# freewym/espresso

Hardware: AMD Instinct MI355X
Metric: audio-hours/sec training (LibriSpeech Conformer-12 + CTC) (higher is better)
Workload: dtype bf16

## Files before the change

espresso_amd/csrc/conv_igemm.hip:

```cpp
#include <hip/hip_runtime.h>

#include "gemm_common.h"

namespace {

typedef const __attribute__((address_space(1))) void* gptr_t;
typedef __attribute__((address_space(3))) void* lptr_t;

struct ConvGatherArgs {
  const bf16_t* src;
  const bf16_t* W;
  bf16_t* out;
  const float* bias;
  double* stats;
  const bf16_t* zero;
  int RB, RT, RF;
  int ST, SF, SC;
  int at, af;
  int ntaps;
  int bt[9], bf[9], koff[9];
  int N;
  long ldw;
  int OT, OF, ot_mul, ot_add, of_mul, of_add;
};

template <int BN_>
__global__ __launch_bounds__(256, 2) void conv_gather_kernel(const ConvGatherArgs a) {
  constexpr int BM_ = 128, NST = 2;
  constexpr int NJ = BN_ / 32;
  constexpr int A_BYTES = BM_ * ROW_BYTES, STAGE = A_BYTES + BN_ * ROW_BYTES;
  constexpr int NA = BM_ / 32, NB = BN_ / 32;
  extern __shared__ __attribute__((aligned(16))) char dsm[];
  const int tid = threadIdx.x, lane = tid & 63, wave = tid >> 6;
  const int wm = wave >> 1, wcol = (wave & 1) * (BN_ / 2);
  const uint32_t M = (uint32_t)a.RB * a.RT * a.RF;
  const uint32_t m0 = blockIdx.x * BM_;
  const int cpt = a.SC / BK;
  const int nk = a.ntaps * cpt;

  int rowb[NA], rowt[NA], rowf[NA];
  int cs[NA];
#pragma unroll
  for (int i = 0; i < NA; ++i) {
    const int r = (wave + 4 * i) * 8 + (lane >> 3);
    cs[i] = (lane & 7) ^ (r & 7) ^ ((r >> 4) & 7);
    const uint32_t p = m0 + r;
    if (p < M) {
      const uint32_t q = p / (uint32_t)a.RF, b = q / (uint32_t)a.RT;
      const int rf = (int)(p - q * a.RF), rt = (int)(q - b * a.RT);
      rowb[i] = (int)b * a.ST;
      rowt[i] = rt * a.at;
      rowf[i] = rf * a.af;
    } else {
      rowb[i] = -1;
      rowt[i] = rowf[i] = 0;
    }
  }
  const bf16_t* bp[NB];
#pragma unroll
  for (int i = 0; i < NB; ++i) {
    const int r = (wave + 4 * i) * 8 + (lane >> 3);
    const int c = (lane & 7) ^ (r & 7) ^ ((r >> 4) & 7);
    bp[i] = a.W + (long)min(r, a.N - 1) * a.ldw + c * 8;
  }
  auto issue = [&](int stage, int kt) {
    const int tap = kt / cpt, chunk = kt - tap * cpt;
    const int dt = a.bt[tap], df = a.bf[tap];
    const long ko = a.koff[tap] + chunk * BK;
    char* base = dsm + stage * STAGE + wave * 1024;
#pragma unroll
    for (int i = 0; i < NA; ++i) {
      const int st = rowt[i] + dt, sf = rowf[i] + df;
      const bool ok = rowb[i] >= 0 && (unsigned)st < (unsigned)a.ST && (unsigned)sf < (unsigned)a.SF;
      const bf16_t* s = ok ? a.src + (((long)(rowb[i] + st)) * a.SF + sf) * a.SC + chunk * BK + cs[i] * 8 : a.zero + cs[i] * 8;
      __builtin_amdgcn_global_load_lds((gptr_t)s, (lptr_t)(base + i * 4096), 16, 0, 0);
    }
#pragma unroll
    for (int i = 0; i < NB; ++i)
      __builtin_amdgcn_global_load_lds((gptr_t)(bp[i] + ko), (lptr_t)(base + A_BYTES + i * 4096), 16, 0, 0);
  };

  f32x4_t acc[4][NJ];
#pragma unroll
// ... 27 lines not shown
      for (int i = 0; i < 4; ++i)
#pragma unroll
        for (int j = 0; j < NJ; ++j)
          acc[i][j] = __builtin_amdgcn_mfma_f32_16x16x32_bf16(
              __builtin_bit_cast(__attribute__((ext_vector_type(8))) __bf16, af[i]),
              __builtin_bit_cast(__attribute__((ext_vector_type(8))) __bf16, bfr[j]), acc[i][j], 0, 0, 0);
    }
    stage ^= 1;
  }

  constexpr int CG = BN_ / 8;
  constexpr int RL = 256 / CG;
  float* sC = reinterpret_cast<float*>(dsm);
  const int cg = tid % CG, rlane = tid / CG;
  float bias8[8], s8[8], q8[8];
#pragma unroll
  for (int e = 0; e < 8; ++e) {
    bias8[e] = a.bias ? a.bias[cg * 8 + e] : 0.f;
    s8[e] = q8[e] = 0.f;
  }
#pragma unroll 1
  for (int half = 0; half < 2; ++half) {
    __syncthreads();
    if (wm == half) {
#pragma unroll
      for (int i = 0; i < 4; ++i)
#pragma unroll
        for (int j = 0; j < NJ; ++j)
#pragma unroll
          for (int r = 0; r < 4; ++r) sC[(i * 16 + (lane >> 4) * 4 + r) * BN_ + wcol + j * 16 + (lane & 15)] = acc[i][j][r];
    }
    __syncthreads();
#pragma unroll 1
    for (int pass = 0; pass < 64 / RL; ++pass) {
      const int rl = pass * RL + rlane;
      const uint32_t p = m0 + half * 64 + rl;
      if (p < M) {
        const uint32_t q = p / (uint32_t)a.RF, b = q / (uint32_t)a.RT;
        const int rf = (int)(p - q * a.RF), rt = (int)(q - b * a.RT);
        const long orow = ((long)b * a.OT + (long)rt * a.ot_mul + a.ot_add) * a.OF + (long)rf * a.of_mul + a.of_add;
        const float4 x0 = *reinterpret_cast<const float4*>(sC + rl * BN_ + cg * 8);
        const float4 x1 = *reinterpret_cast<const float4*>(sC + rl * BN_ + cg * 8 + 4);
        float v[8] = {x0.x, x0.y, x0.z, x0.w, x1.x, x1.y, x1.z, x1.w};
#pragma unroll
        for (int e = 0; e < 8; ++e) v[e] += bias8[e];
        uint4 u;
        u.x = pack_bf2(v[0], v[1]); u.y = pack_bf2(v[2], v[3]); u.z = pack_bf2(v[4], v[5]); u.w = pack_bf2(v[6], v[7]);
        *reinterpret_cast<uint4*>(a.out + orow * a.N + cg * 8) = u;
        if (a.stats) {
          const uint32_t w[4] = {u.x, u.y, u.z, u.w};
#pragma unroll
          for (int e = 0; e < 4; ++e) {
            const float lo = __uint_as_float(w[e] << 16), hi = __uint_as_float(w[e] & 0xffff0000u);
            s8[2 * e] += lo; q8[2 * e] += lo * lo;
            s8[2 * e + 1] += hi; q8[2 * e + 1] += hi * hi;
          }
        }
      }
    }
  }
  if (a.stats) {
    __syncthreads();
    float* red = reinterpret_cast<float*>(dsm);
#pragma unroll
    for (int e = 0; e < 8; ++e) {
      red[(rlane * 2 + 0) * BN_ + cg * 8 + e] = s8[e];
      red[(rlane * 2 + 1) * BN_ + cg * 8 + e] = q8[e];
    }
    __syncthreads();
    if (tid < 2 * BN_) {
      const int which = tid / BN_, c = tid - which * BN_;
      float t = 0.f;
      for (int r = 0; r < RL; ++r) t += red[(r * 2 + which) * BN_ + c];
      atomicAdd(a.stats + which * a.N + c, (double)t);
    }
  }
}

const bf16_t* zero_line(hipStream_t stream) {
  static bf16_t* z = nullptr;
  if (!z) {
    if (hipMalloc(&z, 256) != hipSuccess) return nullptr;
    if (hipMemsetAsync(z, 0, 256, stream) != hipSuccess) return nullptr;
    hipStreamSynchronize(stream);
  }
  return z;
}

template <int BN_>
int launch_gather(const ConvGatherArgs& a, hipStream_t stream) {
  constexpr int bytes = 2 * (128 + BN_) * ROW_BYTES;
  static bool attr_ok = hipFuncSetAttribute(reinterpret_cast<const void*>(&conv_gather_kernel<BN_>),
                                            hipFuncAttributeMaxDynamicSharedMemorySize, bytes) == hipSuccess;
  if (!attr_ok) return -1;
  const long M = (long)a.RB * a.RT * a.RF;
  if (M <= 0) return 0;
  if (M >= (1L << 31) - 128) return -1;
  hipLaunchKernelGGL((conv_gather_kernel<BN_>), dim3((unsigned)((M + 127) / 128)), dim3(256), bytes, stream, a);
  return EA_CHECK_LAUNCH();
}


struct ConvWgradArgs {
  const bf16_t* X;
  const bf16_t* dZ;
  float* slab;
  const bf16_t* zero;
  int RB, RT, RF, ST, SF, Cin, Cout;
  int at, af, ntaps;
  int bt[9], bf[9];
  int chunks_per_wg;
  int ablate;
};

__device__ __forceinline__ int tr_sw(int r) { return (r & 3) ^ ((r >> 3) & 1); }
__device__ __forceinline__ void ds_read_tr16_x8(const uint32_t (&ad)[8], uint2 (&o)[8]) {
// ... 209 lines not shown
  const long chunks = (M + 63) / 64;
  const int blocks = (Cin / 64) * (Cout / 64);
  static const long target = [] { const char* e = getenv("EA_CONV_WGRAD_WGS"); const long v = e ? atol(e) : 0; return v > 0 ? v : 256L; }();
  long nsplit = (target + blocks - 1) / blocks;
  if (nsplit > chunks / 8) nsplit = chunks / 8;
  if (nsplit < 1) nsplit = 1;
  return (int)nsplit;
}

}

extern "C" int ea_conv3x3_fwd(const void* X, const void* W, const float* bias, void* Z, double* stats, int B, int T, int F,
                              int Cin, int Cout, int sy, int sx, hipStream_t stream) {
  if (B <= 0 || T <= 0 || F <= 0) return 0;
  if (Cin % 64 || (Cout != 64 && Cout != 128) || sy < 1 || sx < 1) return -2;
  ConvGatherArgs a;
  a.src = (const bf16_t*)X; a.W = (const bf16_t*)W; a.out = (bf16_t*)Z; a.bias = bias; a.stats = stats;
  a.zero = zero_line(stream);
  if (!a.zero) return -1;
  const int To = (T - 1) / sy + 1, Fo = (F - 1) / sx + 1;
  a.RB = B; a.RT = To; a.RF = Fo;
  a.ST = T; a.SF = F; a.SC = Cin;
  a.at = sy; a.af = sx;
  a.ntaps = 9;
  for (int ky = 0; ky < 3; ++ky)
    for (int kx = 0; kx < 3; ++kx) {
      const int t = ky * 3 + kx;
      a.bt[t] = ky - 1; a.bf[t] = kx - 1; a.koff[t] = t * Cin;
    }
  a.N = Cout; a.ldw = 9L * Cin;
  a.OT = To; a.OF = Fo; a.ot_mul = 1; a.ot_add = 0; a.of_mul = 1; a.of_add = 0;
  return Cout == 128 ? launch_gather<128>(a, stream) : launch_gather<64>(a, stream);
}

extern "C" int ea_conv3x3_dgrad(const void* dZ, const void* Wd, void* dX, int B, int T, int F, int Cin, int Cout, int sy, int sx,
                                hipStream_t stream) {
  if (B <= 0 || T <= 0 || F <= 0) return 0;
  if (Cout % 64 || (Cin != 64 && Cin != 128) || sy < 1 || sx < 1 || sy > 2 || sx > 2) return -2;
  const int To = (T - 1) / sy + 1, Fo = (F - 1) / sx + 1;
  const bf16_t* zero = zero_line(stream);
  if (!zero) return -1;
  for (int pt = 0; pt < sy; ++pt)
    for (int pf = 0; pf < sx; ++pf) {
      ConvGatherArgs a;
      a.src = (const bf16_t*)dZ; a.W = (const bf16_t*)Wd; a.out = (bf16_t*)dX; a.bias = nullptr; a.stats = nullptr; a.zero = zero;
      a.RB = B; a.RT = (T - pt + sy - 1) / sy; a.RF = (F - pf + sx - 1) / sx;
      a.ST = To; a.SF = Fo; a.SC = Cout;
      a.at = 1; a.af = 1;
      a.ntaps = 0;
      for (int ky = 0; ky < 3; ++ky) {
        if ((pt + 1 - ky) % sy) continue;
        for (int kx = 0; kx < 3; ++kx) {
          if ((pf + 1 - kx) % sx) continue;
          const int t = a.ntaps++;
          a.bt[t] = (pt + 1 - ky) / sy; a.bf[t] = (pf + 1 - kx) / sx; a.koff[t] = (ky * 3 + kx) * Cout;
        }
      }
      a.N = Cin; a.ldw = 9L * Cout;
      a.OT = T; a.OF = F; a.ot_mul = sy; a.ot_add = pt; a.of_mul = sx; a.of_add = pf;
      if (a.RT <= 0 || a.RF <= 0) continue;
      if (a.ntaps == 0) return -2;
      const int rc = Cin == 128 ? launch_gather<128>(a, stream) : launch_gather<64>(a, stream);
      if (rc) return rc;
    }
  return 0;
}

extern "C" long ea_conv3x3_wgrad_workspace_bytes(int B, int T, int F, int Cin, int Cout, int sy, int sx) {
  const int To = (T - 1) / sy + 1, Fo = (F - 1) / sx + 1;
  return (long)wgrad_split((long)B * To * Fo, Cin, Cout) * Cout * 9 * Cin * (long)sizeof(float);
}

static int conv3x3_wgrad_impl(const void* X, const void* dZ, float* dW, void* workspace, int B, int T, int F, int Cin, int Cout,
                              int sy, int sx, int param_layout, hipStream_t stream);
extern "C" int ea_conv3x3_wgrad(const void* X, const void* dZ, float* dW, void* workspace, int B, int T, int F, int Cin, int Cout,
                                int sy, int sx, hipStream_t stream) {
  return conv3x3_wgrad_impl(X, dZ, dW, workspace, B, T, F, Cin, Cout, sy, sx, 0, stream);
}
extern "C" int ea_conv3x3_wgrad_param_layout(const void* X, const void* dZ, float* dW, void* workspace, int B, int T, int F, int Cin,
                                             int Cout, int sy, int sx, hipStream_t stream) {
  return conv3x3_wgrad_impl(X, dZ, dW, workspace, B, T, F, Cin, Cout, sy, sx, 1, stream);
// ... 40 lines not shown
```

espresso_amd/csrc/convmodule.hip:

```cpp
#include "common.h"
#include "espresso_amd.h"

namespace {

constexpr int KMAX = 31;

__device__ __forceinline__ float sigmoid_f(float x) { return __builtin_amdgcn_rcpf(1.f + __expf(-x)); }

constexpr int CT = 64, TTILE = 64, TPT = TTILE / 4;

template <int KW>
__global__ __launch_bounds__(256) void glu_dwconv_fwd_kernel(const bf16_t* __restrict__ Y,
                                                             const float* __restrict__ w,
                                                             bf16_t* __restrict__ U, bf16_t* __restrict__ Z,
                                                             double* __restrict__ stats, int T, int C) {
  constexpr int PAD = (KW - 1) / 2, ROWS = TTILE + KW - 1;
  __shared__ __attribute__((aligned(16))) float su[ROWS][CT];
  __shared__ float sred[2][4][CT];
  const int c0 = blockIdx.x * CT, t0 = blockIdx.y * TTILE, b = blockIdx.z;
  const long rowbase = (long)b * T;
  if ((C & 7) == 0 && c0 + CT <= C) {
    bf16_t (*sub)[CT] = reinterpret_cast<bf16_t (*)[CT]>(&su[0][0]);
    bf16_t (*sz)[CT] = reinterpret_cast<bf16_t (*)[CT]>(&su[0][0]) + ROWS;
    constexpr int NCH = (ROWS * (CT / 8) + 255) / 256;
// ... 733 lines not shown
__device__ __forceinline__ int c1_sw(int r) { return (r & 3) ^ ((r >> 3) & 1); }
__device__ __forceinline__ void c1_tr_read8(const uint32_t (&ad)[8], uint2 (&o)[8]) {
  asm volatile(
      "ds_read_b64_tr_b16 %0, %8\n\tds_read_b64_tr_b16 %1, %9\n\tds_read_b64_tr_b16 %2, %10\n\tds_read_b64_tr_b16 %3, %11\n\t"
      "ds_read_b64_tr_b16 %4, %12\n\tds_read_b64_tr_b16 %5, %13\n\tds_read_b64_tr_b16 %6, %14\n\tds_read_b64_tr_b16 %7, %15\n\t"
      "s_waitcnt lgkmcnt(0)"
      : "=&v"(o[0]), "=&v"(o[1]), "=&v"(o[2]), "=&v"(o[3]), "=&v"(o[4]), "=&v"(o[5]), "=&v"(o[6]), "=&v"(o[7])
      : "v"(ad[0]), "v"(ad[1]), "v"(ad[2]), "v"(ad[3]), "v"(ad[4]), "v"(ad[5]), "v"(ad[6]), "v"(ad[7])
      : "memory");
}
__global__ __launch_bounds__(256) void conv1_bn_bwd_wgrad_kernel(const float* __restrict__ X, const bf16_t* __restrict__ Z,
                                                                 const bf16_t* __restrict__ dH, const float* __restrict__ mean_rstd,
                                                                 const float* __restrict__ gamma, const float* __restrict__ beta,
                                                                 const float* __restrict__ red, float* __restrict__ dW,
                                                                 float* __restrict__ dbias, int T, int F, int To, int Fo, int CO,
                                                                 int sy, int sx, long npos, int act, float n) {
  __shared__ __attribute__((aligned(16))) char tile[4][32 * 128];
  __shared__ float sred[4][64][16];
  const int lane = threadIdx.x & 63, wave = threadIdx.x >> 6;
  const int li = lane & 15, g4 = lane >> 4;
  const float invn = n > 0.f ? 1.f / n : 0.f;
  const long nblk = (npos + 31) / 32;
  const long bmax = (npos - 1) / ((long)Fo * To);
  const uint32_t lds0 = (uint32_t)(uintptr_t)(&tile[wave][0]);
  for (int cs = 0; cs < CO; cs += 64) {
    const int c8 = lane & 7, prow = lane >> 3;
    float mu[8], rs[8], ga[8], be[8], r0[8], r1[8];
#pragma unroll
    for (int e = 0; e < 8; ++e) {
      const int c = cs + c8 * 8 + e;
      mu[e] = mean_rstd[c]; rs[e] = mean_rstd[CO + c]; ga[e] = gamma[c]; be[e] = beta[c];
      r0[e] = red[c] * invn; r1[e] = red[CO + c] * invn;
    }
    f32x4_t acc[4];
// ... 141 lines not shown
                               int F, int CO, int sy, int sx, int act, int training, hipStream_t stream) {
  if (B <= 0 || T <= 0) return 0;
  if (CO % 64) return -2;
  const int To = (T - 1) / sy + 1, Fo = (F - 1) / sx + 1;
  const long npos = (long)B * To * Fo;
  launch_bn_bwd_reduce(Z, dH, mean_rstd, gamma, beta, red, npos, CO, act, stream);
  long nb = (npos + 127) / 128;
  if (nb > 1024) nb = 1024;
  hipLaunchKernelGGL(conv1_bn_bwd_wgrad_kernel, dim3((unsigned)nb), dim3(256), 0, stream, X, (const bf16_t*)Z,
                     (const bf16_t*)dH, mean_rstd, gamma, beta, red, dW, dbias, T, F, To, Fo, CO, sy, sx, npos, act,
                     training ? (float)npos : 0.f);
  if (dgamma || dbeta) hipLaunchKernelGGL(bn_param_grad_kernel, dim3((CO + 255) / 256), dim3(256), 0, stream, red, dgamma, dbeta, CO);
  return EA_CHECK_LAUNCH();
}

static void launch_bn_bwd_reduce(const void* Z, const void* dH, const float* mean_rstd, const float* gamma, const float* beta,
                                 float* red, long M, int C, int act, hipStream_t stream) {
  const int nch = C / 8;
  int TCH = 1;
  while (TCH < 256 && TCH < nch) TCH <<= 1;
  const int lanes = 256 / TCH;
  int rpb = 8 * lanes;
  if (rpb < 32) rpb = 32;
  const long gx = (nch + TCH - 1) / TCH;
  const long want = (M + (2048 / gx) - 1) / (2048 / gx > 0 ? 2048 / gx : 1);
  if (want > rpb) rpb = (int)((want + lanes - 1) / lanes * lanes);
  dim3 g1((unsigned)gx, (unsigned)((M + rpb - 1) / rpb));
  hipLaunchKernelGGL(bn_act_bwd_reduce_kernel, g1, dim3(256), (size_t)256 * 16 * sizeof(float), stream, (const bf16_t*)Z,
                     (const bf16_t*)dH, mean_rstd, gamma, beta, red, M, C, act, rpb, TCH);
}
// ... 53 lines not shown
```

espresso_amd/functional.py:

```python
import collections

import ctypes
import os

import torch

from . import kernels as K

_seed_state = {"base": 0x5EED, "counter": 0}


def set_dropout_seed(seed: int):
    _seed_state["base"] = int(seed) & 0xFFFFFFFF
    _seed_state["counter"] = 0


_seed_trace = None


class trace_dropout_seeds:

    def __enter__(self):
        global _seed_trace
        self.prev, self.entries = _seed_trace, []
# ... 641 lines not shown
    return _LabelSmoothedCE.apply(logits, target, pad_idx, eps, smoothing, prior, tgt_len)


_CONV_IGEMM = True


_CONV1_FUSED_BWD = True


def set_conv1_fused_backward(on: bool) -> bool:
    global _CONV1_FUSED_BWD
    old, _CONV1_FUSED_BWD = _CONV1_FUSED_BWD, bool(on)
    return old


def set_conv_implicit_gemm(on: bool):
    global _CONV_IGEMM
    _CONV_IGEMM = bool(on)


def _conv_igemm_ok(cin, cout, sy, sx):
    return _CONV_IGEMM and cin in (64, 128) and cout in (64, 128) and sy in (1, 2) and sx in (1, 2)


class _ConvSubsample(torch.autograd.Function):

    @staticmethod
    def forward(ctx, X, row_zero, strides, bufs, p_drop, training, bn_eps, bn_momentum, *params):
        B, T, F = X.shape
        L = len(params) // 4
# ... 53 lines not shown
        for i in range(L):
            per.append([next(it) if has else None for has in ctx.layout[i]])
        dout = dout.contiguous()
        if seed:
            dout = K.scale_dropout(dout, a=1.0, drop_p=p_drop, drop_seed=seed)
        elif row_zero is not None:
            dout = dout.clone()
        if row_zero is not None:
            K.zero_rows(dout, row_zero)
        grads = [None] * (4 * L)
        Tc, Fc, Cc, To, Fo, Co, sy, sx = cfgs[-1]
        dA = dout.view(B * To * Fo, Co)
        cur = torch.cuda.current_stream(X.device)
        side = _side_stream(X.device)
        keep = []
        for i in range(L - 1, -1, -1):
            Zi, mr, col, w16, g, beta = per[i]
            Tc, Fc, Cc, To, Fo, Co, sy, sx = cfgs[i]
            pw, pb, pg, pbe = ctx.params[4 * i: 4 * i + 4]
            sg, sbe = (_grad_sink(pg, Co), _grad_sink(pbe, Co)) if training else (None, None)
            if sg is not None and sbe is not None:
                dg, dbeta = sg, sbe
            else:
                sg = sbe = None
                dg, dbeta = _zeros_f32(Co, X), _zeros_f32(Co, X)
            if i == 0 and Co % 64 == 0 and _CONV1_FUSED_BWD:
                sW, sb = _grad_sink(pw, Co * 9), _grad_sink(pb, Co)
                if sW is not None and sb is not None:
                    db, dW = sb, sW
                else:
                    sW = None
                    db, dW = _zeros_f32(Co, X), _zeros_f32(Co * 9, X)
                K.conv1_bn_bwd(X, Zi, dA, mr, g, beta, dg, dbeta, dW, db, B, Tc, Fc, Co, sy, sx, "relu", training)
                if sW is None:
                    grads[0], grads[1] = dW.view(wshapes[0]), db
                if sg is None:
                    grads[2], grads[3] = dg, dbeta
                continue
            dZ = K.bn_act_bwd(Zi, dA, mr, g, beta, dg, dbeta, "relu", training)
            keep.append(dZ)
            n = B * To * Fo
            db = _zeros_f32(Co, X)
            if i == 0:
                dW = _zeros_f32(Co * 9, X)
                side.wait_stream(cur)
                with torch.cuda.stream(side):
                    K.conv1_wgrad(X, dZ, dW, db, B, Tc, Fc, Co, sy, sx)
                grads[0] = dW.view(wshapes[0])
            elif ctx.igemm[i]:
                sW = _grad_sink(pw, Co * 9 * Cc)
                side.wait_stream(cur)
                if sW is not None:
                    with torch.cuda.stream(side):
                        K.conv3x3_wgrad(col, dZ, sW, B, Tc, Fc, Cc, Co, sy, sx, param_layout=True)
                else:
                    dWp = _zeros_f32(Co * 9 * Cc, X).view(Co, 9 * Cc)
                    with torch.cuda.stream(side):
                        K.conv3x3_wgrad(col, dZ, dWp, B, Tc, Fc, Cc, Co, sy, sx)
                    grads[4 * i] = dWp.view(Co, 3, 3, Cc).permute(0, 3, 1, 2)
                if not training:
                    db = g.detach() * mr[1] * dbeta
                elif _grad_sink(pb, Co) is not None:
                    db = None
                wd16 = K.cast_f32_to_bf16(ctx.weights[i].detach().permute(1, 2, 3, 0).reshape(Cc, 9 * Co).contiguous())
                dA = K.conv3x3_dgrad(dZ, wd16, B, Tc, Fc, Cc, Co, sy, sx)
            else:
                dWp = torch.empty((Co, 9 * Cc), dtype=torch.float32, device=X.device)
                side.wait_stream(cur)
                with torch.cuda.stream(side):
                    _wgrad(dZ, col, n, Co, 9 * Cc, out=dWp)
                    K.colsum(dZ, db, n, Co, Co)
                grads[4 * i] = dWp.view(Co, 3, 3, Cc).permute(0, 3, 1, 2)
                dcol = _new((n, 9 * Cc), torch.bfloat16, X)
                K.gemm(dZ, w16, dcol, n, 9 * Cc, Co, lda=Co, ldb=9 * Cc, ldc=9 * Cc, b_kstrided=True)
                dA = K.col2im3x3(dcol, B, Tc, Fc, Cc, sy, sx)
            grads[4 * i + 1] = db
            if sg is None:
                grads[4 * i + 2] = dg
                grads[4 * i + 3] = dbeta
        cur.wait_stream(side)
# ... 1303 lines not shown
```

espresso_amd/kernels.py:

```python
import ctypes
from typing import Optional

import torch

from . import _lib
from ._lib import EaGemmParams, check

ACT_NONE, ACT_RELU, ACT_SILU = 0, 1, 2
_ACT = {None: 0, "none": 0, "relu": 1, "silu": 2, "swish": 2}


def _stream():
    return ctypes.c_void_p(torch._C._cuda_getCurrentRawStream(torch._C._cuda_getDevice()))


def _p(t: Optional[torch.Tensor]):
    if t is None:
        return None
    if not t.is_cuda:
        raise RuntimeError("espresso_amd kernels need device tensors (no CPU path)")
    return ctypes.c_void_p(t.data_ptr())


def drop_params(p: float):
# ... 325 lines not shown


def conv3x3_fwd(X, W16, bias, B, T, F, Cin, Cout, sy, sx, stats=None):
    To, Fo = (T - 1) // sy + 1, (F - 1) // sx + 1
    Z = torch.empty((B * To * Fo, Cout), dtype=torch.bfloat16, device=X.device)
    check(_lib.lib().ea_conv3x3_fwd(_p(X), _p(W16), _p(bias), _p(Z), _p(stats), B, T, F, Cin, Cout, sy, sx, _stream()), "ea_conv3x3_fwd")
    return Z


def conv3x3_dgrad(dZ, Wd16, B, T, F, Cin, Cout, sy, sx):
    dX = torch.empty((B * T * F, Cin), dtype=torch.bfloat16, device=dZ.device)
    check(_lib.lib().ea_conv3x3_dgrad(_p(dZ), _p(Wd16), _p(dX), B, T, F, Cin, Cout, sy, sx, _stream()), "ea_conv3x3_dgrad")
    return dX


def conv3x3_wgrad(X, dZ, dW, B, T, F, Cin, Cout, sy, sx, param_layout=False):
    lib = _lib.lib()
    nb = lib.ea_conv3x3_wgrad_workspace_bytes(B, T, F, Cin, Cout, sy, sx)
    ws = torch.empty(nb, dtype=torch.uint8, device=X.device)
    fn = lib.ea_conv3x3_wgrad_param_layout if param_layout else lib.ea_conv3x3_wgrad
    check(fn(_p(X), _p(dZ), _p(dW), _p(ws), B, T, F, Cin, Cout, sy, sx, _stream()), "ea_conv3x3_wgrad")
    return dW


def im2col3x3(A, B, T, F, C, sy, sx):
    To, Fo = (T - 1) // sy + 1, (F - 1) // sx + 1
    col = torch.empty(B * To * Fo, 9 * C, dtype=torch.bfloat16, device=A.device)
    check(_lib.lib().ea_im2col3x3(_p(A), _p(col), B, T, F, C, sy, sx, _stream()), "ea_im2col3x3")
    return col

# ... 382 lines not shown
```

include/espresso_amd.h:

```cpp
#ifndef ESPRESSO_AMD_H
#define ESPRESSO_AMD_H

#include <stdint.h>

#ifdef __cplusplus
extern "C" {
#endif

typedef struct ihipStream_t* ea_stream_t;

int ea_version(void);

enum { EA_ACT_NONE = 0, EA_ACT_RELU = 1, EA_ACT_SILU = 2 };

typedef struct EaGemmParams {
  const void* A;
  const void* B;
  void* C;
  void* C2;
  const float* bias;
  const void* resid;
  const void* aux;
  int M, N, K, batch, zdiv;
  int a_kstrided, b_kstrided, c_f32, accumulate, resid_f32, act;
// ... 137 lines not shown
                      void* wgrad_ws, int B, int T, int C, int KW, ea_stream_t stream);
int ea_dwconv_bwd_weight(const void* dZ, const void* U, float* dw, void* wgrad_ws, int B, int T, int C, int KW, ea_stream_t stream);
int ea_bn_act_fwd_train(const void* Z, const double* stats, float* mean_rstd, float* running_mean, float* running_var,
                        const float* gamma, const float* beta, void* H, long M, int C, int act, float n, float eps,
                        float momentum, double* zero_next, int zero_n, ea_stream_t stream);
int ea_bn_act_bwd_fused(const void* Z, const void* dH, const float* mean_rstd, const float* gamma, const float* beta,
                        float* red, void* dZ, float* dgamma, float* dbeta, long M, int C, int act, int training,
                        float* zero_next, int zero_n, ea_stream_t stream);
int ea_bn_glu_dwconv_bwd_fused(const void* Z, const void* dH, const float* mean_rstd, const float* gamma, const float* beta, float* red,
                               void* dZ, float* dgamma, float* dbeta, int act, int training, float* zero_next, int zero_n,
                               const void* Y, const float* w, void* dY, int B, int T, int C, int KW, ea_stream_t stream);
int ea_bn_param_grad(const float* red, float* dgamma, float* dbeta, int C, ea_stream_t stream);
int ea_conv1_bn_bwd(const float* X, const void* Z, const void* dH, const float* mean_rstd, const float* gamma, const float* beta,
                    float* red, float* dgamma, float* dbeta, float* dW, float* dbias, int B, int T, int F, int CO, int sy, int sx,
                    int act, int training, ea_stream_t stream);

int ea_conv1_fwd(const float* X, const float* W, const float* bias, void* Z, double* stats, int B, int T, int F,
                 int CO, int sy, int sx, ea_stream_t stream);
int ea_conv1_wgrad(const float* X, const void* dZ, float* dW, float* dbias, int B, int T, int F, int CO, int sy,
                   int sx, ea_stream_t stream);
int ea_conv3x3_fwd(const void* X, const void* W, const float* bias, void* Z, double* stats, int B, int T, int F, int Cin,
                   int Cout, int sy, int sx, ea_stream_t stream);
int ea_conv3x3_dgrad(const void* dZ, const void* Wd, void* dX, int B, int T, int F, int Cin, int Cout, int sy, int sx,
                     ea_stream_t stream);
long ea_conv3x3_wgrad_workspace_bytes(int B, int T, int F, int Cin, int Cout, int sy, int sx);
int ea_conv3x3_wgrad(const void* X, const void* dZ, float* dW, void* workspace, int B, int T, int F, int Cin, int Cout, int sy,
                     int sx, ea_stream_t stream);
int ea_conv3x3_wgrad_param_layout(const void* X, const void* dZ, float* dW, void* workspace, int B, int T, int F, int Cin, int Cout,
                                  int sy, int sx, ea_stream_t stream);
int ea_im2col3x3(const void* A, void* col, int B, int T, int F, int C, int sy, int sx, ea_stream_t stream);
int ea_col2im3x3(const void* dcol, void* dA, int B, int T, int F, int C, int sy, int sx, ea_stream_t stream);
int ea_colstats_bf16(const void* X, double* stats, long M, int C, ea_stream_t stream);

int ea_log_softmax_f32(const float* in, long ld_in, float* out, long M, int V, ea_stream_t stream);
int ea_log_softmax_bf16(const void* in, long ld_in, float* out, long M, int V, ea_stream_t stream);
long ea_ctc_workspace_bytes(int B, int T, int Lmax);
int ea_ctc_loss(const float* lprobs, const int* targets, const int* in_len, const int* tgt_len, float* nll,
                void* workspace, int B, int T, int V, int Lmax, int blank, ea_stream_t stream);
int ea_ctc_grad(const float* lprobs, const void* workspace, const float* nll, const int* targets,
// ... 195 lines not shown
```

Before: 5.366.

## Fuse BN backward reductions into strided conv dgrad epilogue and single-launch classes

The strided 3x3 dgrad now runs all parity classes in one launch, with the tap-heavy classes placed first, where it used to launch once per class. Its epilogue also computes the next BatchNorm/ReLU backward partial sums (sum of d and d*xhat) from the freshly produced dX and the saved pre-BN activation. A small fold kernel reduces these per-workgroup partials, and the downstream BN backward and conv1 backward kernels reuse the precomputed sums instead of doing a separate reduction pass over memory. This trades extra Z loads and ALU work in the conv epilogue, plus a workspace buffer, for fewer launches and one fewer full read of the activations.

After: 5.378, median of 6. Within noise of the previous version (+0.2%).

```diff
diff --git a/espresso_amd/csrc/conv_igemm.hip b/espresso_amd/csrc/conv_igemm.hip
--- a/espresso_amd/csrc/conv_igemm.hip
+++ b/espresso_amd/csrc/conv_igemm.hip
@@ -6,6 +6,14 @@
 
 typedef const __attribute__((address_space(1))) void* gptr_t;
 typedef __attribute__((address_space(3))) void* lptr_t;
+
+struct ConvClass {
+  int RT, RF;
+  int ntaps;
+  int ot_add, of_add;
+  int blk0;
+  int bt[9], bf[9], koff[9];
+};
 
 struct ConvGatherArgs {
   const bf16_t* src;
@@ -14,14 +22,20 @@
   const float* bias;
   double* stats;
   const bf16_t* zero;
-  int RB, RT, RF;
+  const bf16_t* bn_Z;
+  const float* bn_mr;
+  const float* bn_g;
+  const float* bn_b;
+  float* bn_part;
+  int bn_act;
+  int RB;
   int ST, SF, SC;
   int at, af;
-  int ntaps;
-  int bt[9], bf[9], koff[9];
   int N;
   long ldw;
-  int OT, OF, ot_mul, ot_add, of_mul, of_add;
+  int OT, OF, ot_mul, of_mul;
+  int ncls;
+  ConvClass cls[4];
 };
 
 template <int BN_>
@@ -33,10 +47,15 @@
   extern __shared__ __attribute__((aligned(16))) char dsm[];
   const int tid = threadIdx.x, lane = tid & 63, wave = tid >> 6;
   const int wm = wave >> 1, wcol = (wave & 1) * (BN_ / 2);
-  const uint32_t M = (uint32_t)a.RB * a.RT * a.RF;
-  const uint32_t m0 = blockIdx.x * BM_;
+  int ci = 0;
+  for (int c = 1; c < a.ncls; ++c)
+    if ((int)blockIdx.x >= a.cls[c].blk0) ci = c;
+  const ConvClass& k = a.cls[ci];
+  const int RT = k.RT, RF = k.RF;
+  const uint32_t M = (uint32_t)a.RB * RT * RF;
+  const uint32_t m0 = (blockIdx.x - k.blk0) * BM_;
   const int cpt = a.SC / BK;
-  const int nk = a.ntaps * cpt;
+  const int nk = k.ntaps * cpt;
 
   int rowb[NA], rowt[NA], rowf[NA];
   int cs[NA];
@@ -46,8 +65,8 @@
     cs[i] = (lane & 7) ^ (r & 7) ^ ((r >> 4) & 7);
     const uint32_t p = m0 + r;
     if (p < M) {
-      const uint32_t q = p / (uint32_t)a.RF, b = q / (uint32_t)a.RT;
-      const int rf = (int)(p - q * a.RF), rt = (int)(q - b * a.RT);
+      const uint32_t q = p / (uint32_t)RF, b = q / (uint32_t)RT;
+      const int rf = (int)(p - q * RF), rt = (int)(q - b * RT);
       rowb[i] = (int)b * a.ST;
       rowt[i] = rt * a.at;
       rowf[i] = rf * a.af;
@@ -65,8 +84,8 @@
   }
   auto issue = [&](int stage, int kt) {
     const int tap = kt / cpt, chunk = kt - tap * cpt;
-    const int dt = a.bt[tap], df = a.bf[tap];
-    const long ko = a.koff[tap] + chunk * BK;
+    const int dt = k.bt[tap], df = k.bf[tap];
+    const long ko = k.koff[tap] + chunk * BK;
     char* base = dsm + stage * STAGE + wave * 1024;
 #pragma unroll
     for (int i = 0; i < NA; ++i) {
@@ -124,13 +143,35 @@
   float* sC = reinterpret_cast<float*>(dsm);
   const int cg = tid % CG, rlane = tid / CG;
   float bias8[8], s8[8], q8[8];
+  float mu[8], rs[8], ga[8], be[8];
 #pragma unroll
   for (int e = 0; e < 8; ++e) {
     bias8[e] = a.bias ? a.bias[cg * 8 + e] : 0.f;
     s8[e] = q8[e] = 0.f;
-  }
+    mu[e] = rs[e] = ga[e] = be[e] = 0.f;
+  }
+  if (a.bn_part) {
+#pragma unroll
+    for (int e = 0; e < 8; ++e) {
+      const int c = cg * 8 + e;
+      mu[e] = a.bn_mr[c]; rs[e] = a.bn_mr[a.N + c]; ga[e] = a.bn_g[c]; be[e] = a.bn_b[c];
+    }
+  }
+  auto out_row = [&](uint32_t p) -> long {
+    const uint32_t q = p / (uint32_t)RF, b = q / (uint32_t)RT;
+    const int rf = (int)(p - q * RF), rt = (int)(q - b * RT);
+    return ((long)b * a.OT + (long)rt * a.ot_mul + k.ot_add) * a.OF + (long)rf * a.of_mul + k.of_add;
+  };
+  constexpr int NP = 64 / RL;
 #pragma unroll 1
   for (int half = 0; half < 2; ++half) {
+    uint4 zpre[NP];
+#pragma unroll
+    for (int pass = 0; pass < NP; ++pass) {
+      zpre[pass] = make_uint4(0, 0, 0, 0);
+      const uint32_t p = m0 + half * 64 + pass * RL + rlane;
+      if (a.bn_part && p < M) zpre[pass] = *reinterpret_cast<const uint4*>(a.bn_Z + out_row(p) * a.N + cg * 8);
+    }
     __syncthreads();
     if (wm == half) {
 #pragma unroll
@@ -141,14 +182,13 @@
           for (int r = 0; r < 4; ++r) sC[(i * 16 + (lane >> 4) * 4 + r) * BN_ + wcol + j * 16 + (lane & 15)] = acc[i][j][r];
     }
     __syncthreads();
-#pragma unroll 1
-    for (int pass = 0; pass < 64 / RL; ++pass) {
+#pragma unroll
+    for (int pass = 0; pass < NP; ++pass) {
       const int rl = pass * RL + rlane;
       const uint32_t p = m0 + half * 64 + rl;
       if (p < M) {
-        const uint32_t q = p / (uint32_t)a.RF, b = q / (uint32_t)a.RT;
-        const int rf = (int)(p - q * a.RF), rt = (int)(q - b * a.RT);
-        const long orow = ((long)b * a.OT + (long)rt * a.ot_mul + a.ot_add) * a.OF + (long)rf * a.of_mul + a.of_add;
+        const long orow = out_row(p);
+        const uint4 uz = zpre[pass];
         const float4 x0 = *reinterpret_cast<const float4*>(sC + rl * BN_ + cg * 8);
         const float4 x1 = *reinterpret_cast<const float4*>(sC + rl * BN_ + cg * 8 + 4);
         float v[8] = {x0.x, x0.y, x0.z, x0.w, x1.x, x1.y, x1.z, x1.w};
@@ -165,11 +205,23 @@
             s8[2 * e] += lo; q8[2 * e] += lo * lo;
             s8[2 * e + 1] += hi; q8[2 * e + 1] += hi * hi;
           }
+        } else if (a.bn_part) {
+          const uint32_t wz[4] = {uz.x, uz.y, uz.z, uz.w}, wd[4] = {u.x, u.y, u.z, u.w};
+#pragma unroll
+          for (int e = 0; e < 8; ++e) {
+            const float z = (e & 1) ? __uint_as_float(wz[e >> 1] & 0xffff0000u) : __uint_as_float(wz[e >> 1] << 16);
+            float d = (e & 1) ? __uint_as_float(wd[e >> 1] & 0xffff0000u) : __uint_as_float(wd[e >> 1] << 16);
+            const float xh = (z - mu[e]) * rs[e];
+            const float y = xh * ga[e] + be[e];
+            d *= a.bn_act == 2 ? dsilu_f(y) : (a.bn_act == 1 ? (y > 0.f ? 1.f : 0.f) : 1.f);
+            s8[e] += d;
+            q8[e] += d * xh;
+          }
         }
       }
     }
   }
-  if (a.stats) {
+  if (a.stats || a.bn_part) {
     __syncthreads();
     float* red = reinterpret_cast<float*>(dsm);
 #pragma unroll
@@ -182,8 +234,25 @@
       const int which = tid / BN_, c = tid - which * BN_;
       float t = 0.f;
       for (int r = 0; r < RL; ++r) t += red[(r * 2 + which) * BN_ + c];
-      atomicAdd(a.stats + which * a.N + c, (double)t);
-    }
+      if (a.stats) atomicAdd(a.stats + which * a.N + c, (double)t);
+      else a.bn_part[(long)blockIdx.x * 2 * BN_ + tid] = t;
+    }
+  }
+}
+
+__global__ __launch_bounds__(256) void conv_bn_sums_fold_kernel(const float* __restrict__ part, float* __restrict__ red, int nwg, int C2,
+                                                                int per) {
+  __shared__ float sm[256];
+  const int lanes = 256 / C2, col = threadIdx.x % C2, ln = threadIdx.x / C2;
+  const int w0 = blockIdx.x * per, w1 = min(nwg, w0 + per);
+  float t = 0.f;
+  if (ln < lanes)
+    for (int w = w0 + ln; w < w1; w += lanes) t += part[(long)w * C2 + col];
+  sm[threadIdx.x] = t;
+  __syncthreads();
+  if (threadIdx.x < C2) {
+    for (int l = 1; l < lanes; ++l) t += sm[l * C2 + threadIdx.x];
+    atomicAdd(red + threadIdx.x, t);
   }
 }
 
@@ -198,18 +267,70 @@
 }
 
 template <int BN_>
-int launch_gather(const ConvGatherArgs& a, hipStream_t stream) {
+int launch_gather(ConvGatherArgs a, bool single, hipStream_t stream) {
   constexpr int bytes = 2 * (128 + BN_) * ROW_BYTES;
   static bool attr_ok = hipFuncSetAttribute(reinterpret_cast<const void*>(&conv_gather_kernel<BN_>),
                                             hipFuncAttributeMaxDynamicSharedMemorySize, bytes) == hipSuccess;
   if (!attr_ok) return -1;
-  const long M = (long)a.RB * a.RT * a.RF;
-  if (M <= 0) return 0;
-  if (M >= (1L << 31) - 128) return -1;
-  hipLaunchKernelGGL((conv_gather_kernel<BN_>), dim3((unsigned)((M + 127) / 128)), dim3(256), bytes, stream, a);
-  return EA_CHECK_LAUNCH();
-}
-
+  long nblk = 0;
+  for (int c = 0; c < a.ncls; ++c) {
+    const long M = (long)a.RB * a.cls[c].RT * a.cls[c].RF;
+    if (M >= (1L << 31) - 128) return -1;
+    a.cls[c].blk0 = (int)nblk;
+    nblk += (M + 127) / 128;
+  }
+  if (nblk <= 0) return 0;
+  if (nblk >= (1L << 31) / 128) return -1;
+  if (single || a.ncls == 1) {
+    hipLaunchKernelGGL((conv_gather_kernel<BN_>), dim3((unsigned)nblk), dim3(256), bytes, stream, a);
+    return EA_CHECK_LAUNCH();
+  }
+  for (int c = 0; c < a.ncls; ++c) {
+    ConvGatherArgs one = a;
+    one.ncls = 1;
+    one.cls[0] = a.cls[c];
+    one.cls[0].blk0 = 0;
+    const long n = (c + 1 < a.ncls ? a.cls[c + 1].blk0 : nblk) - a.cls[c].blk0;
+    if (a.bn_part) one.bn_part = a.bn_part + (long)a.cls[c].blk0 * 2 * BN_;
+    if (n <= 0) continue;
+    hipLaunchKernelGGL((conv_gather_kernel<BN_>), dim3((unsigned)n), dim3(256), bytes, stream, one);
+    const int rc = EA_CHECK_LAUNCH();
+    if (rc) return rc;
+  }
+  return 0;
+}
+
+int dgrad_classes(ConvGatherArgs& a, int T, int F, int Cout, int sy, int sx, bool most_taps_first) {
+  a.ncls = 0;
+  for (int pt = 0; pt < sy; ++pt)
+    for (int pf = 0; pf < sx; ++pf) {
+      ConvClass k{};
+      k.RT = (T - pt + sy - 1) / sy; k.RF = (F - pf + sx - 1) / sx;
+      k.ot_add = pt; k.of_add = pf;
+      for (int ky = 0; ky < 3; ++ky) {
+        if ((pt + 1 - ky) % sy) continue;
+        for (int kx = 0; kx < 3; ++kx) {
+          if ((pf + 1 - kx) % sx) continue;
+          const int t = k.ntaps++;
+          k.bt[t] = (pt + 1 - ky) / sy; k.bf[t] = (pf + 1 - kx) / sx; k.koff[t] = (ky * 3 + kx) * Cout;
+        }
+      }
+      if (k.RT <= 0 || k.RF <= 0) continue;
+      if (k.ntaps == 0) return -2;
+      a.cls[a.ncls++] = k;
+    }
+  if (most_taps_first)
+    for (int i = 1; i < a.ncls; ++i)
+      for (int j = i; j > 0 && a.cls[j].ntaps > a.cls[j - 1].ntaps; --j) {
+        const ConvClass t = a.cls[j]; a.cls[j] = a.cls[j - 1]; a.cls[j - 1] = t;
+      }
+  return a.ncls;
+}
+
+bool subsample_bwd_fused() {
+  static const bool on = [] { const char* e = getenv("EA_SUBSAMPLE_BWD_FUSED"); return !(e && e[0] == '0'); }();
+  return on;
+}
 
 struct ConvWgradArgs {
   const bf16_t* X;
@@ -449,57 +570,83 @@
                               int Cin, int Cout, int sy, int sx, hipStream_t stream) {
   if (B <= 0 || T <= 0 || F <= 0) return 0;
   if (Cin % 64 || (Cout != 64 && Cout != 128) || sy < 1 || sx < 1) return -2;
-  ConvGatherArgs a;
+  ConvGatherArgs a{};
   a.src = (const bf16_t*)X; a.W = (const bf16_t*)W; a.out = (bf16_t*)Z; a.bias = bias; a.stats = stats;
   a.zero = zero_line(stream);
   if (!a.zero) return -1;
   const int To = (T - 1) / sy + 1, Fo = (F - 1) / sx + 1;
-  a.RB = B; a.RT = To; a.RF = Fo;
+  a.RB = B;
   a.ST = T; a.SF = F; a.SC = Cin;
   a.at = sy; a.af = sx;
-  a.ntaps = 9;
+  a.ncls = 1;
+  ConvClass& k = a.cls[0];
+  k.RT = To; k.RF = Fo; k.ntaps = 9; k.ot_add = 0; k.of_add = 0;
   for (int ky = 0; ky < 3; ++ky)
     for (int kx = 0; kx < 3; ++kx) {
       const int t = ky * 3 + kx;
-      a.bt[t] = ky - 1; a.bf[t] = kx - 1; a.koff[t] = t * Cin;
+      k.bt[t] = ky - 1; k.bf[t] = kx - 1; k.koff[t] = t * Cin;
     }
   a.N = Cout; a.ldw = 9L * Cin;
-  a.OT = To; a.OF = Fo; a.ot_mul = 1; a.ot_add = 0; a.of_mul = 1; a.of_add = 0;
-  return Cout == 128 ? launch_gather<128>(a, stream) : launch_gather<64>(a, stream);
+  a.OT = To; a.OF = Fo; a.ot_mul = 1; a.of_mul = 1;
+  return Cout == 128 ? launch_gather<128>(a, true, stream) : launch_gather<64>(a, true, stream);
+}
+
+static int conv3x3_dgrad_impl(const void* dZ, const void* Wd, void* dX, int B, int T, int F, int Cin, int Cout, int sy, int sx,
+                              bool single, const void* Zbn, const float* mean_rstd, const float* gamma, const float* beta, int act,
+                              float* red, float* part, hipStream_t stream) {
+  if (B <= 0 || T <= 0 || F <= 0) return 0;
+  if (Cout % 64 || (Cin != 64 && Cin != 128) || sy < 1 || sx < 1 || sy > 2 || sx > 2) return -2;
+  ConvGatherArgs a{};
+  a.src = (const bf16_t*)dZ; a.W = (const bf16_t*)Wd; a.out = (bf16_t*)dX; a.bias = nullptr; a.stats = nullptr;
+  a.zero = zero_line(stream);
+  if (!a.zero) return -1;
+  const int To = (T - 1) / sy + 1, Fo = (F - 1) / sx + 1;
+  a.RB = B;
+  a.ST = To; a.SF = Fo; a.SC = Cout;
+  a.at = 1; a.af = 1;
+  a.N = Cin; a.ldw = 9L * Cout;
+  a.OT = T; a.OF = F; a.ot_mul = sy; a.of_mul = sx;
+  if (dgrad_classes(a, T, F, Cout, sy, sx, single) < 0) return -2;
+  const bool bn = Zbn != nullptr;
+  if (bn) {
+    if (!mean_rstd || !gamma || !beta || !red || !part) return -2;
+    a.bn_Z = (const bf16_t*)Zbn; a.bn_mr = mean_rstd; a.bn_g = gamma; a.bn_b = beta; a.bn_part = part; a.bn_act = act;
+  }
+  const int rc = Cin == 128 ? launch_gather<128>(a, single, stream) : launch_gather<64>(a, single, stream);
+  if (rc || !bn) return rc;
+  long nwg = 0;
+  for (int c = 0; c < a.ncls; ++c) nwg += ((long)B * a.cls[c].RT * a.cls[c].RF + 127) / 128;
+  if (nwg <= 0) return 0;
+  const int per = (int)((nwg + 255) / 256) < 8 ? 8 : (int)((nwg + 255) / 256);
+  hipLaunchKernelGGL(conv_bn_sums_fold_kernel, dim3((unsigned)((nwg + per - 1) / per)), dim3(256), 0, stream, (const float*)part, red,
+                     (int)nwg, 2 * Cin, per);
+  return EA_CHECK_LAUNCH();
 }
 
 extern "C" int ea_conv3x3_dgrad(const void* dZ, const void* Wd, void* dX, int B, int T, int F, int Cin, int Cout, int sy, int sx,
                                 hipStream_t stream) {
-  if (B <= 0 || T <= 0 || F <= 0) return 0;
-  if (Cout % 64 || (Cin != 64 && Cin != 128) || sy < 1 || sx < 1 || sy > 2 || sx > 2) return -2;
-  const int To = (T - 1) / sy + 1, Fo = (F - 1) / sx + 1;
-  const bf16_t* zero = zero_line(stream);
-  if (!zero) return -1;
+  return conv3x3_dgrad_impl(dZ, Wd, dX, B, T, F, Cin, Cout, sy, sx, subsample_bwd_fused(), nullptr, nullptr, nullptr, nullptr, 0,
+                            nullptr, nullptr, stream);
+}
+
+extern "C" int ea_conv3x3_dgrad_ex(const void* dZ, const void* Wd, void* dX, int B, int T, int F, int Cin, int Cout, int sy, int sx,
+                                   int single_launch, const void* Zbn, const float* mean_rstd, const float* gamma, const float* beta,
+                                   int act, float* red, float* part, hipStream_t stream) {
+  return conv3x3_dgrad_impl(dZ, Wd, dX, B, T, F, Cin, Cout, sy, sx, single_launch != 0, Zbn, mean_rstd, gamma, beta, act, red, part,
+                            stream);
+}
+
+extern "C" long ea_conv3x3_dgrad_bn_workspace_bytes(int B, int T, int F, int Cin, int sy, int sx) {
+  long nwg = 0;
   for (int pt = 0; pt < sy; ++pt)
     for (int pf = 0; pf < sx; ++pf) {
-      ConvGatherArgs a;
-      a.src = (const bf16_t*)dZ; a.W = (const bf16_t*)Wd; a.out = (bf16_t*)dX; a.bias = nullptr; a.stats = nullptr; a.zero = zero;
-      a.RB = B; a.RT = (T - pt + sy - 1) / sy; a.RF = (F - pf + sx - 1) / sx;
-      a.ST = To; a.SF = Fo; a.SC = Cout;
-      a.at = 1; a.af = 1;
-      a.ntaps = 0;
-      for (int ky = 0; ky < 3; ++ky) {
-        if ((pt + 1 - ky) % sy) continue;
-        for (int kx = 0; kx < 3; ++kx) {
-          if ((pf + 1 - kx) % sx) continue;
-          const int t = a.ntaps++;
-          a.bt[t] = (pt + 1 - ky) / sy; a.bf[t] = (pf + 1 - kx) / sx; a.koff[t] = (ky * 3 + kx) * Cout;
-        }
-      }
-      a.N = Cin; a.ldw = 9L * Cout;
-      a.OT = T; a.OF = F; a.ot_mul = sy; a.ot_add = pt; a.of_mul = sx; a.of_add = pf;
-      if (a.RT <= 0 || a.RF <= 0) continue;
-      if (a.ntaps == 0) return -2;
-      const int rc = Cin == 128 ? launch_gather<128>(a, stream) : launch_gather<64>(a, stream);
-      if (rc) return rc;
-    }
-  return 0;
-}
+      const long rt = (T - pt + sy - 1) / sy, rf = (F - pf + sx - 1) / sx;
+      if (rt > 0 && rf > 0) nwg += ((long)B * rt * rf + 127) / 128;
+    }
+  return nwg * 2 * Cin * (long)sizeof(float);
+}
+
+extern "C" int ea_subsample_bwd_fused(void) { return subsample_bwd_fused() ? 1 : 0; }
 
 extern "C" long ea_conv3x3_wgrad_workspace_bytes(int B, int T, int F, int Cin, int Cout, int sy, int sx) {
   const int To = (T - 1) / sy + 1, Fo = (F - 1) / sx + 1;
diff --git a/espresso_amd/csrc/convmodule.hip b/espresso_amd/csrc/convmodule.hip
--- a/espresso_amd/csrc/convmodule.hip
+++ b/espresso_amd/csrc/convmodule.hip
@@ -771,10 +771,16 @@
                                                                  const float* __restrict__ gamma, const float* __restrict__ beta,
                                                                  const float* __restrict__ red, float* __restrict__ dW,
                                                                  float* __restrict__ dbias, int T, int F, int To, int Fo, int CO,
-                                                                 int sy, int sx, long npos, int act, float n) {
+                                                                 int sy, int sx, long npos, int act, float n,
+                                                                 float* __restrict__ dgamma = nullptr, float* __restrict__ dbeta = nullptr) {
   __shared__ __attribute__((aligned(16))) char tile[4][32 * 128];
   __shared__ float sred[4][64][16];
   const int lane = threadIdx.x & 63, wave = threadIdx.x >> 6;
+  if (blockIdx.x == 0 && (dgamma || dbeta))
+    for (int c = threadIdx.x; c < CO; c += 256) {
+      if (dbeta) dbeta[c] += red[c];
+      if (dgamma) dgamma[c] += red[CO + c];
+    }
   const int li = lane & 15, g4 = lane >> 4;
   const float invn = n > 0.f ? 1.f / n : 0.f;
   const long nblk = (npos + 31) / 32;
@@ -946,6 +952,31 @@
   return EA_CHECK_LAUNCH();
 }
 
+extern "C" int ea_bn_act_bwd_apply(const void* Z, const void* dH, const float* mean_rstd, const float* gamma, const float* beta,
+                                   const float* red, void* dZ, float* dgamma, float* dbeta, long M, int C, int act, int training,
+                                   hipStream_t stream) {
+  if (M <= 0) return 0;
+  if (C % 8) return -2;
+  hipLaunchKernelGGL(bn_act_bwd_apply_kernel, dim3(egrid_ch(M * (C / 8), C / 8)), dim3(256), 0, stream, (const bf16_t*)Z,
+                     (const bf16_t*)dH, mean_rstd, gamma, beta, red, (bf16_t*)dZ, M, C, act, training ? (float)M : 0.f, dgamma, dbeta,
+                     nullptr, 0);
+  return EA_CHECK_LAUNCH();
+}
+extern "C" int ea_conv1_bn_bwd_sums(const float* X, const void* Z, const void* dH, const float* mean_rstd, const float* gamma,
+                                    const float* beta, const float* red, float* dgamma, float* dbeta, float* dW, float* dbias, int B,
+                                    int T, int F, int CO, int sy, int sx, int act, int training, hipStream_t stream) {
+  if (B <= 0 || T <= 0) return 0;
+  if (CO % 64) return -2;
+  const int To = (T - 1) / sy + 1, Fo = (F - 1) / sx + 1;
+  const long npos = (long)B * To * Fo;
+  long nb = (npos + 127) / 128;
+  if (nb > 1024) nb = 1024;
+  hipLaunchKernelGGL(conv1_bn_bwd_wgrad_kernel, dim3((unsigned)nb), dim3(256), 0, stream, X, (const bf16_t*)Z,
+                     (const bf16_t*)dH, mean_rstd, gamma, beta, red, dW, dbias, T, F, To, Fo, CO, sy, sx, npos, act,
+                     training ? (float)npos : 0.f, dgamma, dbeta);
+  return EA_CHECK_LAUNCH();
+}
+
 static void launch_bn_bwd_reduce(const void* Z, const void* dH, const float* mean_rstd, const float* gamma, const float* beta,
                                  float* red, long M, int C, int act, hipStream_t stream) {
   const int nch = C / 8;
diff --git a/espresso_amd/functional.py b/espresso_amd/functional.py
--- a/espresso_amd/functional.py
+++ b/espresso_amd/functional.py
@@ -679,6 +679,19 @@
     return old
 
 
+_SUBSAMPLE_BWD_FUSED = None
+
+
+def set_subsample_fused_backward(on) -> bool:
+    global _SUBSAMPLE_BWD_FUSED
+    old, _SUBSAMPLE_BWD_FUSED = _subsample_bwd_fused(), (None if on is None else bool(on))
+    return old
+
+
+def _subsample_bwd_fused():
+    return K.subsample_bwd_fused() if _SUBSAMPLE_BWD_FUSED is None else _SUBSAMPLE_BWD_FUSED
+
+
 def set_conv_implicit_gemm(on: bool):
     global _CONV_IGEMM
     _CONV_IGEMM = bool(on)
@@ -762,6 +775,8 @@
         cur = torch.cuda.current_stream(X.device)
         side = _side_stream(X.device)
         keep = []
+        fused = _subsample_bwd_fused()
+        red = None
         for i in range(L - 1, -1, -1):
             Zi, mr, col, w16, g, beta = per[i]
             Tc, Fc, Cc, To, Fo, Co, sy, sx = cfgs[i]
@@ -779,13 +794,20 @@
                 else:
                     sW = None
                     db, dW = _zeros_f32(Co, X), _zeros_f32(Co * 9, X)
-                K.conv1_bn_bwd(X, Zi, dA, mr, g, beta, dg, dbeta, dW, db, B, Tc, Fc, Co, sy, sx, "relu", training)
+                if red is not None:
+                    K.conv1_bn_bwd_sums(X, Zi, dA, mr, g, beta, red, dg, dbeta, dW, db, B, Tc, Fc, Co, sy, sx, "relu", training)
+                else:
+                    K.conv1_bn_bwd(X, Zi, dA, mr, g, beta, dg, dbeta, dW, db, B, Tc, Fc, Co, sy, sx, "relu", training)
                 if sW is None:
                     grads[0], grads[1] = dW.view(wshapes[0]), db
                 if sg is None:
                     grads[2], grads[3] = dg, dbeta
                 continue
-            dZ = K.bn_act_bwd(Zi, dA, mr, g, beta, dg, dbeta, "relu", training)
+            if red is not None:
+                dZ = K.bn_act_bwd_apply(Zi, dA, mr, g, beta, red, dg, dbeta, "relu", training)
+                red = None
+            else:
+                dZ = K.bn_act_bwd(Zi, dA, mr, g, beta, dg, dbeta, "relu", training)
             keep.append(dZ)
             n = B * To * Fo
             db = _zeros_f32(Co, X)
@@ -811,7 +833,12 @@
                 elif _grad_sink(pb, Co) is not None:
                     db = None
                 wd16 = K.cast_f32_to_bf16(ctx.weights[i].detach().permute(1, 2, 3, 0).reshape(Cc, 9 * Co).contiguous())
-                dA = K.conv3x3_dgrad(dZ, wd16, B, Tc, Fc, Cc, Co, sy, sx)
+                if fused:
+                    Zp, mrp, _, _, gp, bep = per[i - 1]
+                    dA, red = K.conv3x3_dgrad_bn(dZ, wd16, B, Tc, Fc, Cc, Co, sy, sx, Zp, mrp, gp, bep, "relu")
+                    keep += [Zp]
+                else:
+                    dA, _ = K.conv3x3_dgrad_bn(dZ, wd16, B, Tc, Fc, Cc, Co, sy, sx, None, None, None, None, None, single_launch=False)
             else:
                 dWp = torch.empty((Co, 9 * Cc), dtype=torch.float32, device=X.device)
                 side.wait_stream(cur)
diff --git a/espresso_amd/kernels.py b/espresso_amd/kernels.py
--- a/espresso_amd/kernels.py
+++ b/espresso_amd/kernels.py
@@ -363,6 +363,38 @@
     return dX
 
 
+def conv3x3_dgrad_bn(dZ, Wd16, B, T, F, Cin, Cout, sy, sx, Zbn, mean_rstd, gamma, beta, act, single_launch=True):
+    from . import functional as _F
+
+    lib = _lib.lib()
+    dX = torch.empty((B * T * F, Cin), dtype=torch.bfloat16, device=dZ.device)
+    red = part = None
+    if Zbn is not None:
+        red = _F._pool_zeros((2, Cin), torch.float32, dZ.device)
+        part = torch.empty(int(lib.ea_conv3x3_dgrad_bn_workspace_bytes(B, T, F, Cin, sy, sx)) // 4, dtype=torch.float32, device=dZ.device)
+    check(lib.ea_conv3x3_dgrad_ex(_p(dZ), _p(Wd16), _p(dX), B, T, F, Cin, Cout, sy, sx, int(bool(single_launch)), _p(Zbn),
+                                  _p(mean_rstd), _p(gamma), _p(beta), _ACT[act], _p(red), _p(part), _stream()), "ea_conv3x3_dgrad_ex")
+    return dX, red
+
+
+def bn_act_bwd_apply(Z, dH, mean_rstd, gamma, beta, red, dgamma, dbeta, act, training=True):
+    M, C = Z.shape
+    dZ = torch.empty_like(Z)
+    check(_lib.lib().ea_bn_act_bwd_apply(_p(Z), _p(dH), _p(mean_rstd), _p(gamma), _p(beta), _p(red), _p(dZ), _p(dgamma), _p(dbeta),
+                                         M, C, _ACT[act], int(training), _stream()), "ea_bn_act_bwd_apply")
+    return dZ
+
+
+def conv1_bn_bwd_sums(X, Z, dH, mean_rstd, gamma, beta, red, dgamma, dbeta, dW, dbias, B, T, F, CO, sy, sx, act, training=True):
+    check(_lib.lib().ea_conv1_bn_bwd_sums(_p(X), _p(Z), _p(dH), _p(mean_rstd), _p(gamma), _p(beta), _p(red), _p(dgamma), _p(dbeta),
+                                          _p(dW), _p(dbias), B, T, F, CO, sy, sx, _ACT[act], int(training), _stream()),
+          "ea_conv1_bn_bwd_sums")
+
+
+def subsample_bwd_fused():
+    return bool(_lib.lib().ea_subsample_bwd_fused())
+
+
 def conv3x3_wgrad(X, dZ, dW, B, T, F, Cin, Cout, sy, sx, param_layout=False):
     lib = _lib.lib()
     nb = lib.ea_conv3x3_wgrad_workspace_bytes(B, T, F, Cin, Cout, sy, sx)
diff --git a/include/espresso_amd.h b/include/espresso_amd.h
--- a/include/espresso_amd.h
+++ b/include/espresso_amd.h
@@ -175,6 +175,11 @@
 int ea_conv1_bn_bwd(const float* X, const void* Z, const void* dH, const float* mean_rstd, const float* gamma, const float* beta,
                     float* red, float* dgamma, float* dbeta, float* dW, float* dbias, int B, int T, int F, int CO, int sy, int sx,
                     int act, int training, ea_stream_t stream);
+int ea_bn_act_bwd_apply(const void* Z, const void* dH, const float* mean_rstd, const float* gamma, const float* beta, const float* red,
+                        void* dZ, float* dgamma, float* dbeta, long M, int C, int act, int training, ea_stream_t stream);
+int ea_conv1_bn_bwd_sums(const float* X, const void* Z, const void* dH, const float* mean_rstd, const float* gamma, const float* beta,
+                         const float* red, float* dgamma, float* dbeta, float* dW, float* dbias, int B, int T, int F, int CO, int sy,
+                         int sx, int act, int training, ea_stream_t stream);
 
 int ea_conv1_fwd(const float* X, const float* W, const float* bias, void* Z, double* stats, int B, int T, int F,
                  int CO, int sy, int sx, ea_stream_t stream);
@@ -184,6 +189,11 @@
                    int Cout, int sy, int sx, ea_stream_t stream);
 int ea_conv3x3_dgrad(const void* dZ, const void* Wd, void* dX, int B, int T, int F, int Cin, int Cout, int sy, int sx,
                      ea_stream_t stream);
+int ea_conv3x3_dgrad_ex(const void* dZ, const void* Wd, void* dX, int B, int T, int F, int Cin, int Cout, int sy, int sx,
+                        int single_launch, const void* Zbn, const float* mean_rstd, const float* gamma, const float* beta, int act,
+                        float* red, float* part, ea_stream_t stream);
+long ea_conv3x3_dgrad_bn_workspace_bytes(int B, int T, int F, int Cin, int sy, int sx);
+int ea_subsample_bwd_fused(void);
 long ea_conv3x3_wgrad_workspace_bytes(int B, int T, int F, int Cin, int Cout, int sy, int sx);
 int ea_conv3x3_wgrad(const void* X, const void* dZ, float* dW, void* workspace, int B, int T, int F, int Cin, int Cout, int sy,
                      int sx, ea_stream_t stream);
```
